# felixchenfy/Monocular-Visual-Odometry

Measured on AMD Instinct MI355X. Metric: frames/sec (extract+match+5-kf BA), 640x480 / 2000 kp, 1->8 MI355X, higher is better.
Workload: dtype u8 (extract/match) + f64 (BA); 1 GPU

## Files before the change

### include/mvo_hip.h

```cpp
#ifndef MVO_HIP_H
#define MVO_HIP_H
#include <stdint.h>

#ifdef __cplusplus
extern "C" {
#endif

#define MVO_OK 0
#define MVO_ERR_INVALID (-1)
#define MVO_ERR_NO_DEVICE (-2)
#define MVO_ERR_CAPACITY (-3)
#define MVO_ERR_HIP (-4)
#define MVO_ERR_STATE (-5)

typedef struct mvo_ctx mvo_ctx;

typedef struct {
    float x, y, size, angle, response;
    int32_t octave, class_id;
} mvo_keypoint;

typedef struct {
    int32_t queryIdx, trainIdx, imgIdx;
    float distance;
// ... 206 lines not shown
    double R[9], t[3], T_w_c[16], mean_depth, scale;
    double mean_pixel_dist, mean_angle, median_angle, min_angle, max_angle;
    int criteria[3], good;
} mvo_init_result;
int mvo_init_two_view(mvo_ctx* ctx, const float* pts1, const float* pts2, int n, double fx, double fy, double cx,
                      double cy, double prob, double threshold, double h_threshold, double h_confidence, double sigma,
                      const double* T_w_c_ref, const mvo_init_params* params, mvo_init_poses* poses,
                      mvo_init_result* out);
int mvo_retain_good_triangulation(const float* pts3d_in_curr, int n, const double* T_w_c_curr, const double* T_w_c_ref,
                                  double min_triang_angle, double max_ratio_to_median, int32_t* keep, int* n_keep,
                                  double* angles);
int mvo_rodrigues(const double* rvec, double* R);
int mvo_invert_pose(const double* T, double* T_inv);

int mvo_ba_launch_stats(int device, long long* launches, long long* windows, double* ms, int reset);
int mvo_debug_ba_service_times(int device, double* out5);
int mvo_debug_ba_resident_stats(int device, long long* windows, long long* grid_starts);
int mvo_debug_ba_resident_cycles(int device, double* shader_cycles);
int mvo_debug_ba_path_switches(int device, long long* n);
int mvo_debug_ba_demand_replay(const double* times, int n, uint8_t* decisions);
int mvo_profile_enable(mvo_ctx* ctx, int on);
int mvo_profile_reset(mvo_ctx* ctx);
typedef struct {
    char name[48];
    int64_t launches;
    double total_ms;
} mvo_kernel_time;
int mvo_profile_get(mvo_ctx* ctx, mvo_kernel_time* out, int cap);

int mvo_debug_set(const char* key, int value);
int mvo_debug_ba_trace_enable(mvo_ctx* ctx, int on);
int mvo_debug_get_ba_trace(mvo_ctx* ctx, mvo_ba_handle* handle, double* rows, int cap, int* n);
int mvo_debug_get_ba_plan(mvo_ctx* ctx, mvo_ba_handle* handle, int* wgs, int* nsplit, int32_t* wg_pt_start, int cap);
int mvo_debug_get_ba_phases(mvo_ctx* ctx, long long* cycles, int n, int* wgs);
int mvo_debug_get_level(mvo_ctx* ctx, int level, int blurred, uint8_t* out, int cap, int* w, int* h, int* stride);
int mvo_debug_get_candidates(mvo_ctx* ctx, void* out, int cap, int* n);
int mvo_debug_get_undistort_map(mvo_ctx* ctx, int32_t* ix, int32_t* iy, uint8_t* ax, uint8_t* ay, int cap);

int mvo_debug_get_pnp(mvo_ctx* ctx, double* models, int32_t* counts, int cap, int32_t* info);

int mvo_debug_get_essential(mvo_ctx* ctx, int32_t* counts, int cap_iters, int32_t* info);

int mvo_debug_get_homography(mvo_ctx* ctx, int32_t* counts, int cap_iters, int32_t* info);

int mvo_debug_get_recover_pose(mvo_ctx* ctx, int32_t* good, int32_t* chosen, double* R1R2t, uint8_t* masks, int cap);
int mvo_debug_get_homography_decomposition(mvo_ctx* ctx, double* Hn, double* w, int32_t* branch, double* Rs,
                                           double* ts, double* normals, int32_t* rejected);
int mvo_debug_get_init_finish(mvo_ctx* ctx, float* p_curr, double* cosang, double* pixdist, int cap, int* n);

#ifdef __cplusplus
}
#endif
#endif
```

### monocular-visual-odometry_amd/__init__.py

```python
import ctypes as C
import os

import numpy as np

from . import synth

_HERE = os.path.dirname(os.path.abspath(__file__))
LIB_PATH = os.path.join(_HERE, "csrc", "libmvo_hip.so")
HEADER_PATH = os.path.join(os.path.dirname(_HERE), "include", "mvo_hip.h")

MVO_OK, MVO_ERR_INVALID, MVO_ERR_NO_DEVICE, MVO_ERR_CAPACITY, MVO_ERR_HIP, MVO_ERR_STATE = 0, -1, -2, -3, -4, -5

KEYPOINT_DTYPE = np.dtype([("x", "<f4"), ("y", "<f4"), ("size", "<f4"), ("angle", "<f4"),
                           ("response", "<f4"), ("octave", "<i4"), ("class_id", "<i4")])
DMATCH_DTYPE = np.dtype([("queryIdx", "<i4"), ("trainIdx", "<i4"), ("imgIdx", "<i4"), ("distance", "<f4")])
CANDIDATE_DTYPE = np.dtype([("x", "<i2"), ("y", "<i2"), ("level_score", "<i4"), ("harris", "<f4"), ("angle", "<f4")])
DISTRIBUTE_CANDIDATE_DTYPE = np.dtype([("x", "<i4"), ("y", "<i4"), ("level", "<i4"), ("score", "<i4")])


class OrbParams(C.Structure):
    _fields_ = [("nfeatures", C.c_int32), ("scale_factor", C.c_float), ("nlevels", C.c_int32),
                ("fast_threshold", C.c_int32), ("max_keypoints", C.c_int32), ("grid_size", C.c_int32),
                ("grid_max_per_cell", C.c_int32), ("pyramid_interpolation", C.c_int32)]

# ... 456 lines not shown

    def ba_solve_batch(self, problems, **kw):
        prs = (BaProblem * len(problems))()
        keeps = []
        for i, a in enumerate(problems):
            d = dict(info=(1, 0, 0, 1), huber_delta=1.0, fix_points=False, pose_fixed=None, max_iterations=50)
            d.update(kw)
            pr, keep = self._ba_problem(*a, d["info"], d["huber_delta"], d["fix_points"], d["pose_fixed"], d["max_iterations"])
            prs[i] = pr
            keeps.append(keep)
        sts = (BaStats * len(problems))()
        self._chk(self.lib.mvo_ba_solve_batch(self.h, prs, len(problems), sts))
        return [(k["poses"].reshape(-1, 4, 4), k["points"], {f: getattr(sts[i], f) for f, _ in BaStats._fields_})
                for i, k in enumerate(keeps)]

    def ba_set_mode(self, mode):
        self._chk(self.lib.mvo_ba_set_mode(self.h, {"latency": 0, "throughput": 1, "shared": 2}[mode]))

    def ba_trace_enable(self, on=True):
        self._chk(self.lib.mvo_debug_ba_trace_enable(self.h, int(on)))

    def ba_trace(self, handle=None, raw_rows=0):
        out = np.zeros((512, 4))
        n = C.c_int()
        self._chk(self.lib.mvo_debug_get_ba_trace(self.h, handle[0] if handle else None, _p(out),
                                                  -int(raw_rows) if raw_rows else 512, C.byref(n)))
        return out[:n.value].copy()

    def ba_plan(self, handle=None):
        g, ns = C.c_int(), C.c_int()
        pt = np.zeros(257, np.int32)
        self._chk(self.lib.mvo_debug_get_ba_plan(self.h, handle[0] if handle else None, C.byref(g), C.byref(ns), _p(pt), 257))
        return dict(wgs=g.value, nsplit=ns.value & 0xffff, groups=max(1, ns.value >> 16), wg_pt_start=pt[:g.value + 1].copy())

    def map_create(self):
        m = C.c_void_p()
        self._chk(self.lib.mvo_map_create(self.h, C.byref(m)))
        return m

    def map_release(self, m):
        self.lib.mvo_map_release.restype = None
        self.lib.mvo_map_release(self.h, m)

    def map_upload(self, m, pos, desc):
        pos = np.ascontiguousarray(pos, np.float32).reshape(-1, 3)
        desc = np.ascontiguousarray(desc, np.uint8).reshape(-1, 32)
        assert len(pos) == len(desc)
        self._chk(self.lib.mvo_map_upload(self.h, m, _p(pos), _p(desc), len(pos)))

    def map_update_positions(self, m, pos, first=0):
        pos = np.ascontiguousarray(pos, np.float32).reshape(-1, 3)
        self._chk(self.lib.mvo_map_update_positions(self.h, m, _p(pos), int(first), len(pos)))

    def map_points_in_view(self, m, T_w_c, K, cols, rows, cap):
        T = np.ascontiguousarray(T_w_c, np.float64).reshape(4, 4)
        idx = np.zeros(max(cap, 1), np.int32)
        px = np.zeros((max(cap, 1), 2), np.float32)
        n = C.c_int()
        d = C.c_void_p()
        self._chk(self.lib.mvo_map_points_in_view(self.h, m, _p(T), C.c_double(K["fx"]), C.c_double(K["fy"]),
                                                  C.c_double(K["cx"]), C.c_double(K["cy"]), int(cols), int(rows),
                                                  _p(idx), _p(px), int(cap), C.byref(n), C.byref(d)))
        return idx[:n.value].copy(), px[:n.value].copy(), d.value

    def solve_pnp_ransac(self, pts3d, pts2d, K, iterations=100, reprojection_error=2.0, confidence=0.999):
        p3 = np.ascontiguousarray(pts3d, np.float32).reshape(-1, 3)
# ... 435 lines not shown
```

### monocular-visual-odometry_amd/csrc/ba_host.cpp

```cpp
#include <algorithm>
#include <atomic>
#include <cmath>
#include <cstdio>
#include <condition_variable>
#include <cstdlib>
#include <cstring>
#include <chrono>
#include <deque>
#include <map>
#include <mutex>
#include <thread>
#include <vector>

#include "ba_types.h"
#include "mvo_internal.h"

int ba_kernel_set_lds_limit();
hipError_t ba_kernel_launch(const BaBatch& batch, int max_wgs, size_t lds_bytes, hipStream_t stream, int profile, int nr, int slots);
int ba_solver_class(int n);
hipError_t ba_service_launch(const BaServiceArgs& a, hipStream_t stream);

void ba_service_free(int device, void* p, bool host);

int g_ba_use_mfma = 1;
// ... 5 lines not shown
int g_ba_service = 1;
int g_ba_edge_rows = -1;
int g_ba_uv_global = std::getenv("MVO_BA_UV_GLOBAL") ? std::atoi(std::getenv("MVO_BA_UV_GLOBAL")) : 1;
int g_ba_chunk_pieces = 0;
int g_ba_block_solver = 0;
int g_ba_groups = std::getenv("MVO_BA_GROUPS") ? std::atoi(std::getenv("MVO_BA_GROUPS")) : 1;
int g_ba_alias_sl = std::getenv("MVO_BA_ALIAS_SL") ? std::atoi(std::getenv("MVO_BA_ALIAS_SL")) : 1;

struct BaDemand {
    double t[128] = {0}, flip = -1e9, low_since = -1, last = 0, rate_avg = 0;
    long long n = 0, total = 0, flips = 0;
    bool on = false;
    bool submit(double now);
};

namespace {

struct Carver {
    size_t off = 0;
    size_t take(size_t bytes) {
        size_t o = off;
        off = (off + bytes + 255) / 256 * 256;
        return o;
    }
};

struct BaPlan {
    int F = 0, L = 0, E = 0, G = 1, nfree = 0, n = 0, NT = 1, npair = 1, nlow = 0, npk = 16, slice = 0, nsplit = 1, npar = 1, nseq = 1,
        ldu = 16, nhp = 1, maxEg = 0, maxLg = 0, max_dup = 0, fix_points = 0, e2_edges = 0, slots = 1, npt = 1, panel = 0, uv_global = 0,
        alias_sl = 0, groups = 1;
    bool service = false;
    size_t uarea = 0;
    size_t lds = 0;
    std::vector<int> wg_pt;
    size_t o_desc = 0, o_pin = 0, o_ptsin = 0, o_wpt = 0, o_wed = 0, o_wps = 0, o_ep = 0, o_el = 0, o_uv = 0, o_ptstart = 0,
           o_ptl = 0, o_eof = 0, o_dup = 0, o_slot = 0, o_sp = 0, o_pkt = 0, upload_end = 0, x_end = 0;
    size_t o_uvd = 0, o_dxl = 0, o_stats = 0, o_pout = 0, o_pts = 0, o_xp = 0, o_xr = 0, o_xh = 0, o_xc = 0, total = 0;
    size_t m_stats = 0, m_poses = 0, m_pts = 0, m_trace = 0, pin_total = 0;
    bool runnable = true;
};

struct BaWorkspace {
    int device = 0;
    char* dev = nullptr;
    size_t dev_cap = 0;
    char* pin = nullptr;
    size_t pin_cap = 0;
    unsigned seq = 0;
    size_t x_sig[5] = {0, 0, 0, 0, 0};
    hipEvent_t ready = nullptr;
    BaPlan plan;
    bool in_flight = false;
    bool poisoned = false;
};

int ws_reserve(mvo_ctx* ctx, BaWorkspace& ws, size_t dev_bytes, size_t pin_bytes) {
    ws.device = ctx->device;
    if (ws.poisoned) {
        ws.dev = ws.pin = nullptr;
        ws.dev_cap = ws.pin_cap = 0;
        ws.seq = 0;
        std::memset(ws.x_sig, 0, sizeof ws.x_sig);
        ws.poisoned = false;
    }
    if (!ws.ready) MVO_HIP(hipEventCreateWithFlags(&ws.ready, hipEventDisableTiming));
    if (dev_bytes > ws.dev_cap) {
// ... 703 lines not shown
                P.panel = (n + 1 > 32 || g_ba_block_solver) ? 1 : 0;
                uarea = ba_uarea_doubles(do_schur ? 4 * npar * msplit : 0, ldu, pt_edges, maxEpose, nhp, G, p->fix_points);
                const bool uv_may_be_global = !all_lds && maxEg > BA_THREADS && g_ba_uv_global;
                for (int uvg = 0; uvg <= (uv_may_be_global ? 1 : 0) && !fits; ++uvg) {
                    P.uv_global = uvg;
                    P.alias_sl = (do_schur && npar == 1 && g_ba_alias_sl && uarea >= ba_solver_matrix_doubles(n, nlow + nhp, G, npair, npar)) ? 1 : 0;
                    P.lds = ba_lds_bytes(F, n, nlow, nhp, G, npair, npar, nfree, maxEg, maxLg, p->fix_points, uarea, P.e2_edges, P.panel, P.uv_global,
                                         P.alias_sl);
                    fits = P.lds <= BA_LDS_BUDGET;
                }
                if (plan_trace)
                    std::fprintf(stderr, "[mvo plan] G %d rows_in_lds %d chunks %d pieces %d pt_passes %d maxEg %d maxLg %d uarea %zu B lds %zu B (budget %d) %s\n",
                                 G, all_lds, nseq, npar, P.npt, maxEg, maxLg, uarea * 8, P.lds, BA_LDS_BUDGET, fits ? "fits" : "-");
                if (all_lds && g_ba_edge_rows != 0) {
                    if (uarea < (size_t)BA_MSTRIDE * (maxEg + 2 * F)) fits = false;
                    break;
                }
            }
        }
        if (fits && maxEg <= BA_EDGE_SLOTS * BA_THREADS && maxLg < 32000) break;
        if (G >= BA_MAX_WGS)
            return mvo_set_err(ctx, MVO_ERR_CAPACITY, "BA window too large for the LDS-resident solver", hipSuccess);
        {
            int next = BA_MAX_WGS;
            for (int c : {2, 4, 8, 16, 32, 64, 128, 256, per_xcd / 2, per_xcd, 2 * per_xcd, 4 * per_xcd, 8 * per_xcd})
                if (c > G && c < next) next = c;
            G = next;
        }
    }
    g_stage_times.lap(0);
    P.nsplit = nsplit;
    P.npar = npar;
    P.nseq = nseq;
    P.uarea = uarea;
    P.G = G;
    P.maxEg = maxEg;
    P.maxLg = maxLg;
    P.groups = 1;
    if (G > 32 && g_ba_groups) {
        int K = 2;
        while (G / K > 32 && K < 8) K *= 2;
        if (G % K == 0 && G / K <= 32 && uarea >= (size_t)K * (size_t)(nlow + nhp)) P.groups = K;
    }
    P.slice = (nlow + G / P.groups - 1) / (G / P.groups);
    std::vector<int>&e_pose = SC.e_pose, &e_point = SC.e_point, &ptstart = SC.ptstart, &ptlist = SC.ptlist;
    std::vector<double>& e_uv = SC.e_uv;
    e_pose.resize(E);
    e_point.resize(E);
    ptstart.assign(L + 1, 0);
    ptlist.resize(E);
    e_uv.resize(2 * (size_t)E);
    {
        std::vector<int>& cur = SC.cur;
        cur.resize((size_t)G * std::max(F, 1));
        for (int g = 0; g < G; ++g)
            for (int q = 0; q < F; ++q) cur[(size_t)g * F + q] = wg_pose[(size_t)g * (F + 1) + q];
        for (int e : act) {
            const int k = cur[(size_t)owner[p->edge_point[e]] * F + p->edge_pose[e]]++;
            e_pose[k] = p->edge_pose[e];
            e_point[k] = p->edge_point[e];
            e_uv[2 * (size_t)k] = p->edge_uv[2 * (size_t)e];
            e_uv[2 * (size_t)k + 1] = p->edge_uv[2 * (size_t)e + 1];
        }
    }
    for (int k = 0; k < E; ++k) ptstart[e_point[k] + 1]++;
    for (int i = 0; i < L; ++i) ptstart[i + 1] += ptstart[i];
    {
        std::vector<int>& cur = SC.cur2;
        cur.assign(ptstart.begin(), ptstart.end() - 1);
        for (int k = 0; k < E; ++k) ptlist[cur[e_point[k]]++] = k;
    }
    std::vector<short>&eof = SC.eof, &dup = SC.dup;
    eof.assign((size_t)std::max(L, 1) * std::max(nfree, 1), -1);
    dup.assign(std::max(E, 1), 0);
    int max_dup = 0;
// ... 346 lines not shown
int ba_fetch_device(mvo_ctx* ctx, mvo_ba_handle* H, double* poses, double* points, mvo_ba_stats* st) {
    if (H->ws.plan.runnable) {
        if (!H->launched) return mvo_set_err(ctx, MVO_ERR_STATE, "mvo_ba_fetch without mvo_ba_solve_resident", hipSuccess);
        service_wait(service_for(ctx->device), &H->job, 1);
        H->launched = false;
    }
    return ba_collect(ctx, H->ws, H->job, poses, points, st);
}
void ba_release_device(mvo_ctx* ctx, mvo_ba_handle* H) {
    if (!H) return;
    if (H->launched) service_wait(service_for(ctx ? ctx->device : H->ws.device), &H->job, 1);
    ws_free(H->ws);
    delete H;
}

int ba_get_trace(mvo_ctx* ctx, mvo_ba_handle* H, double* rows, int cap, int* n) {
    BaWorkspace* ws = H ? &H->ws : (ctx->ba_pool && !ctx->ba_pool->ws.empty() ? ctx->ba_pool->ws[0] : nullptr);
    if (!ws || !ws->pin) return mvo_set_err(ctx, MVO_ERR_STATE, "no bundle adjustment has run", hipSuccess);
    const BaStatsDev* s = (const BaStatsDev*)(ws->pin + ws->plan.m_stats);
    const int m = cap < 0 ? std::min(-cap, BA_TRACE_MAX) : std::min(std::min(s->trials, BA_TRACE_MAX), cap);
    if (rows) std::memcpy(rows, ws->pin + ws->plan.m_trace, (size_t)m * sizeof(BaTraceRow));
    if (n) *n = m;
    return MVO_OK;
}
int ba_get_plan(mvo_ctx* ctx, mvo_ba_handle* H, int* G, int* nsplit, int32_t* wg_pt, int cap) {
    BaWorkspace* ws = H ? &H->ws : (ctx->ba_pool && !ctx->ba_pool->ws.empty() ? ctx->ba_pool->ws[0] : nullptr);
    if (!ws) return mvo_set_err(ctx, MVO_ERR_STATE, "no bundle adjustment has been planned", hipSuccess);
    if (G) *G = ws->plan.G;
    if (nsplit) *nsplit = ws->plan.nsplit | (ws->plan.groups > 1 ? ws->plan.groups << 16 : 0);
    if (wg_pt)
        for (int i = 0; i <= ws->plan.G && i < cap; ++i) wg_pt[i] = ws->plan.wg_pt[i];
    return MVO_OK;
}
void ba_service_times(int device, double* out5) {
    for (int i = 0; i < 5; ++i) out5[i] = 0;
    if (device < 0 || device >= 16) return;
    BaService* sp;
    {
        std::lock_guard<std::mutex> lk(*g_service_start);
        sp = g_service[device & 15];
    }
    if (!sp) return;
    std::lock_guard<std::mutex> lk(sp->m);
    out5[0] = sp->t_idle, out5[1] = sp->t_batch, out5[2] = sp->t_launch, out5[3] = sp->t_sync, out5[4] = sp->t_post;
}
void ba_service_park(int device) {
    if (device < 0 || device >= 16) return;
    BaService* sp;
    {
        std::lock_guard<std::mutex> lk(*g_service_start);
        sp = g_service[device & 15];
    }
    if (!sp) return;
    std::unique_lock<std::mutex> lk(sp->m);
    if (!sp->resident) return;
    sp->park_requested = true;
    sp->cv_work.notify_all();
    sp->cv_done.wait_for(lk, std::chrono::milliseconds(50), [&] { return !sp->resident || sp->slots_busy > 0 || !sp->q.empty(); });
}
void ba_resident_stats(int device, long long* windows, long long* grid_starts, double* cycles, long long* path_switches) {
    if (windows) *windows = 0;
    if (grid_starts) *grid_starts = 0;
    if (cycles) *cycles = 0;
    if (path_switches) *path_switches = 0;
    if (device < 0 || device >= 16) return;
    BaService* sp;
// ... 43 lines not shown
```

### monocular-visual-odometry_amd/csrc/ba_kernels.hip

```cpp
#include "ba_types.h"
#include "mvo_internal.h"

typedef ba_u64 u64;
#ifndef MVO_KERNEL_SIM
typedef __attribute__((address_space(1))) double gdouble;
typedef __attribute__((address_space(1))) const u64 gcu64;
typedef __attribute__((address_space(1))) u64 gu64;
#define BA_AS_GLOBAL_D(p) ((gdouble*)(p))
#define BA_AS_GLOBAL_CU64(p) ((gcu64*)(p))
#define BA_AS_GLOBAL_U64(p) ((gu64*)(p))
#else
typedef double gdouble;
typedef const u64 gcu64;
typedef u64 gu64;
#define BA_AS_GLOBAL_D(p) (p)
#define BA_AS_GLOBAL_CU64(p) (p)
#define BA_AS_GLOBAL_U64(p) (p)
#endif

#define PH_BEGIN() long long ph_t = PROF ? (long long)__builtin_amdgcn_s_memtime() : 0
#define PH_END(id)                                                       \
    do {                                                                 \
        if (PROF) {                                                      \
            long long ph_n = (long long)__builtin_amdgcn_s_memtime();    \
// ... 794 lines not shown
    if (do_schur && wave < B.npair * npar) {
#pragma unroll
        for (int j = 0; j < 4; ++j) pk4[j] = pkt_g[(wave % B.npair) * 256 + ((lane >> 4) + 4 * j) * 16 + (lane & 15)];
    }
    EdgeRegs er;
#pragma unroll
    for (int c = 0; c < 6; ++c) er.a0[c] = er.a1[c] = er.x[c] = 0;
    const bool have0 = SLOTS > 0 && tid < Eg, have1 = SLOTS > 1 && tid + BA_THREADS < Eg;
    const int e0_p = have0 ? W.epose[tid] : 0, e0_l = have0 ? W.ept[tid] : 0, e0_sl = have0 ? sSlot[e0_p] : -1;
    constexpr int nslot = SLOTS;
    constexpr int e2_first = SLOTS == 0 ? 0 : BA_THREADS;
#define BA_EDGE_FROM_LDS(BODY, el_)                                          \
    do {                                                                     \
        EdgeRegs r1_;                                                        \
        double ee_[2];                                                       \
        const double* q_ = W.E2 + BA_E2S * ((el_)-e2_first);                 \
        _Pragma("unroll") for (int c_ = 0; c_ < 6; ++c_) {                   \
            r1_.a0[c_] = q_[c_];                                             \
            r1_.a1[c_] = q_[6 + c_];                                         \
            r1_.x[c_] = q_[12 + c_];                                         \
        }                                                                    \
        ee_[0] = q_[18];                                                     \
        ee_[1] = q_[19];                                                     \
        const int p1_ = W.epose[el_];                                        \
        (void)p1_;                                                           \
        BODY(el_, r1_, W.ept[el_], sSlot[p1_], ee_)                          \
    } while (0);
#define BA_EDGES(BODY)                                                       \
    if (nslot > 0 && have0) do { BODY(tid, er, e0_l, e0_sl, ee0) } while (0); \
    if (nslot > 1 && have1) BA_EDGE_FROM_LDS(BODY, tid + BA_THREADS)         \
    if (nslot == 0)                                                          \
        for (int el0_ = tid; el0_ < Eg; el0_ += BA_THREADS) BA_EDGE_FROM_LDS(BODY, el0_)

    int hp_npass = 1;
    {
        const int mcap = (int)(B.uarea / BA_MSTRIDE);
        for (;; ++hp_npass) {
            int tot = 0;
            for (int p = 0; p < B.F; ++p) {
                const int n_p = sPoseStart[p + 1] - sPoseStart[p];
                tot += min(n_p, ((n_p + hp_npass - 1) / hp_npass + 1) & ~1);
            }
            if (tot <= mcap) break;
            if (hp_npass > Eg) {
                error = 1;
                break;
            }
        }
    }
    const bool hp_tables = hp_npass <= BA_HP_PASSES;
    auto hp_slice_row = [&](int q, int row) {
        if (tid < B.F) {
            int off = 0, lo = 0, hi = 0;
            for (int pp = 0; pp <= tid; ++pp) {
                const int s0 = sPoseStart[pp], n_p = sPoseStart[pp + 1] - s0;
                const int h = ((n_p + hp_npass - 1) / hp_npass + 1) & ~1;
                off += hi - lo;
                lo = min(s0 + q * h, s0 + n_p);
                hi = min(s0 + (q + 1) * h, s0 + n_p);
            }
            sSlc[0][row][tid] = (short)lo;
            sSlc[1][row][tid] = (short)hi;
            sSlc[2][row][tid] = (short)off;
        }
    };
    if (hp_tables && !error)
        for (int q = 0; q < hp_npass; ++q) hp_slice_row(q, q);
    int nfp = 0, hp_pa0 = -1, hp_pb0 = -1, hp_pa1 = -1, hp_pb1 = -1;
    for (int p = 0; p < B.F; ++p) {
        if (sSlot[p] < 0) continue;
        if (nfp == 2 * wave) hp_pa0 = p;
        if (nfp == 2 * wave + 1) hp_pb0 = p;
        if (nfp == 2 * (wave + BA_WAVES)) hp_pa1 = p;
        if (nfp == 2 * (wave + BA_WAVES) + 1) hp_pb1 = p;
        ++nfp;
    }
    __syncthreads();

    int piv_hoff = 0;
    if (NR == 32 && n > 0) {
        const int lsh = NR == 32 ? 4 : (n <= 32 ? 4 : (n <= 64 ? 3 : 2)), LPR = 1 << lsh, jj = tid & (LPR - 1);
        const int qi = min(tid >> lsh, n - 1), q0 = min(jj, n - 1), q1 = min(jj + LPR, n - 1);
        piv_hoff = (36 * sSlotPose[qi / 6] + 7 * (qi % 6)) | (36 * sSlotPose[q0 / 6] + 7 * (q0 % 6)) << 10 | (36 * sSlotPose[q1 / 6] + 7 * (q1 % 6)) << 20;
    }
    for (it = 0; any_free && !error && it < B.max_it; ++it) {
        PH_BEGIN();
        BA_PHASE_HEAD();
        double ee0[2] = {0, 0};
// ... 80 lines not shown
                    for (int i = 0; i < 6; ++i) W.Hll[BA_XS * l + i] = h6[i];
#pragma unroll
                    for (int i = 0; i < 3; ++i) W.bl[3 * l + i] = b[i];
                    maxdiag = fmax(maxdiag, fmax(fabs(h6[0]), fmax(fabs(h6[3]), fabs(h6[5]))));
                }
                __syncthreads();
            }
        }
        PH_END(2);
        const bool hp_deferred = do_schur && G > 1 && it > 0;
        const bool hp_local = hp_deferred || G == 1;
        if (!hp_deferred) ++tagH;
        BA_PHASE_HEAD();
        {
            const int col = lane & 15;
            v4d accp0 = {0, 0, 0, 0}, accp1 = {0, 0, 0, 0};
            for (int q = 0; q < hp_npass && !error; ++q) {
                const int tq = hp_tables ? q : 0;
                if (!hp_tables) {
                    hp_slice_row(q, 0);
                    __syncthreads();
                }
#define BA_BODY_STAGE_M(el, r, l_, sl_, ee)                                   \
    const int p_ = W.epose[el];                                              \
    const int lo_ = sSlc[0][tq][p_], hi_ = sSlc[1][tq][p_];                  \
    if ((el) < lo_ || (el) >= hi_) break;                                    \
    double* Mr = stage + BA_MSTRIDE * (sSlc[2][tq][p_] + (el)-lo_);          \
    _Pragma("unroll") for (int c = 0; c < 6; ++c) {                          \
        Mr[c] = r.a0[c];                                                     \
        Mr[7 + c] = r.a1[c];                                                 \
    }                                                                        \
    Mr[6] = ee[0];                                                           \
    Mr[13] = ee[1];
                BA_EDGES(BA_BODY_STAGE_M)
                __syncthreads();
                const bool lastq = q == hp_npass - 1;
                if (batch.use_mfma) {
                    int ai = 0;
                    for (int pair = wave; 2 * pair < nfp; pair += BA_WAVES, ++ai) {
                        const int pa = ai == 0 ? hp_pa0 : hp_pa1, pb = ai == 0 ? hp_pb0 : hp_pb1;
                        const bool second = col >= 8;
                        const int pp = second ? pb : pa;
                        const int cc7 = col & 7;
                        const bool cv = cc7 < 7 && pp >= 0;
                        const int rowsA = 2 * (sSlc[1][tq][pa] - sSlc[0][tq][pa]);
                        const int rowsB = pb >= 0 ? 2 * (sSlc[1][tq][pb] - sSlc[0][tq][pb]) : 0;
                        const int s = pp >= 0 ? sSlc[2][tq][pp] : 0, rows = second ? rowsB : rowsA;
                        const int rmax = max(rowsA, rowsB);
                        const double* pm = stage + BA_MSTRIDE * (s + (lane >> 5)) + 7 * ((lane >> 4) & 1) + (cv ? cc7 : 0);
                        const int kq = lane >> 4;
                        const int myrows = cv ? rows - kq : 0;
                        v4d acc = ai == 0 ? accp0 : accp1;
                        int st = 0;
#define BA_HP_LOAD4(V)                                                                   \
    V##0 = 4 * st < myrows ? pm[0] : 0.0, V##1 = 4 * st + 4 < myrows ? pm[2 * BA_MSTRIDE] : 0.0, \
    V##2 = 4 * st + 8 < myrows ? pm[4 * BA_MSTRIDE] : 0.0, V##3 = 4 * st + 12 < myrows ? pm[6 * BA_MSTRIDE] : 0.0; \
    pm += 8 * BA_MSTRIDE;                                                                \
    st += 4
#define BA_HP_MFMA4_LOADNEXT(V, Wn, more)                                      \
    acc = __builtin_amdgcn_mfma_f64_16x16x4f64(V##0, V##0, acc, 0, 0, 0);       \
    __builtin_amdgcn_sched_barrier(0);                                          \
    if (more) { BA_HP_LOAD4(Wn); }                                              \
    __builtin_amdgcn_sched_barrier(0);                                          \
    acc = __builtin_amdgcn_mfma_f64_16x16x4f64(V##1, V##1, acc, 0, 0, 0);       \
    acc = __builtin_amdgcn_mfma_f64_16x16x4f64(V##2, V##2, acc, 0, 0, 0);       \
    acc = __builtin_amdgcn_mfma_f64_16x16x4f64(V##3, V##3, acc, 0, 0, 0)
                        if (4 * (st + 4) <= rmax) {
                            double a0, a1, a2, a3, c0 = 0, c1 = 0, c2 = 0, c3 = 0;
                            BA_HP_LOAD4(a);
                            for (;;) {
                                const bool more1 = 4 * (st + 4) <= rmax;
                                BA_HP_MFMA4_LOADNEXT(a, c, more1);
                                if (!more1) break;
                                const bool more2 = 4 * (st + 4) <= rmax;
                                BA_HP_MFMA4_LOADNEXT(c, a, more2);
                                if (!more2) break;
                            }
                        }
#undef BA_HP_LOAD4
#undef BA_HP_MFMA4_LOADNEXT
                        for (; 4 * st < rmax; ++st) {
                            const double v = 4 * st < myrows ? pm[0] : 0.0;
                            acc = __builtin_amdgcn_mfma_f64_16x16x4f64(v, v, acc, 0, 0, 0);
                            pm += 2 * BA_MSTRIDE;
                        }
                        if (ai == 0) accp0 = acc;
                        else accp1 = acc;
                        if (lastq) {
#pragma unroll
                            for (int j = 0; j < 4; ++j) {
                                const int rg = (lane >> 4) + 4 * j;
                                const bool mine = second ? (rg >= 8 && rg < 15 && pb >= 0) : rg < 7;
                                const int r7 = rg & 7;
                                if (mine && cc7 <= r7 && cc7 < 7) {
                                    const int sl = sSlot[pp], pk = r7 * (r7 + 1) / 2 + cc7;
                                    if (hp_local) W.hpl[BA_HP * sl + pk] = acc[j];
                                    else gstore_d(B.xH + 2 * ((size_t)g * B.nhp + BA_HP * sl + pk), tag0 + tagH, acc[j], same_l2);
                                }
                            }
                        }
                    }
                } else {
                    for (int p = wave; p < B.F; p += BA_WAVES) {
                        const int sl = sSlot[p];
                        if (sl < 0 || lane >= BA_HP) continue;
                        const int lo = sSlc[0][tq][p], hi = sSlc[1][tq][p];
                        const int s = sSlc[2][tq][p], e = s + hi - lo;
                        int i = 0;
                        while ((i + 1) * (i + 2) / 2 <= lane) ++i;
                        const int j = lane - i * (i + 1) / 2;
                        double acc = q == 0 ? 0.0 : W.hpl[BA_HP * sl + lane];
                        for (int r = 2 * s; r < 2 * e; ++r)
                            acc = __builtin_fma(stage[BA_MSTRIDE * (r >> 1) + 7 * (r & 1) + i], stage[BA_MSTRIDE * (r >> 1) + 7 * (r & 1) + j], acc);
                        if (hp_local || !lastq) W.hpl[BA_HP * sl + lane] = acc;
                        else gstore_d(B.xH + 2 * ((size_t)g * B.nhp + BA_HP * sl + lane), tag0 + tagH, acc, same_l2);
                    }
                }
                __syncthreads();
            }
        }
        PH_END(1);
        BA_PHASE_HEAD();
        if (!hp_deferred) {
            const double m = block_max(maxdiag, sScr);
            const int nhp = B.nhp, hrows = min(G, max(1, (int)(B.uarea / nhp)));
            double hsum = 0, mm = 0;
            if (G > 1) {
                if (tid == 0) gstore_d(B.xH + 2 * ((size_t)g * nhp + nhp - 1), tag0 + tagH, m, same_l2);
                for (int w0 = 0; w0 < G; w0 += hrows) {
                    const int nr = min(hrows, G - w0);
                    if (!gather_tagged(B.xH + 2 * (size_t)w0 * nhp, nr * nhp, nhp, nhp, tag0 + tagH, stage)) sFlag[2] = 1;
                    __syncthreads();
                    if (tid < nhp - 1) {
#pragma unroll 8
                        for (int w = 0; w < nr; ++w) hsum += stage[w * nhp + tid];
                    }
                    if (tid < nr) mm = fmax(mm, stage[tid * nhp + nhp - 1]);
                    __syncthreads();
                }
                if (sFlag[2]) error = 1;
            } else {
                if (tid < nhp - 1) hsum = W.hpl[tid];
                if (tid == 0) mm = m;
            }
            if (tid < BA_HP * nfree) {
                const int sl = tid / BA_HP, pk = tid - BA_HP * sl, p = sSlotPose[sl];
// ... 734 lines not shown
```

### monocular-visual-odometry_amd/csrc/ba_types.h

```cpp
#ifndef MVO_BA_TYPES_H
#define MVO_BA_TYPES_H
#include <stddef.h>
#include <stdint.h>

typedef unsigned long long ba_u64;

#define BA_THREADS 512
#define BA_WAVES 8
#define BA_MAX_POSES 20
#define BA_MSTRIDE 15
#define BA_XS 7
#define BA_SXS 9
#define BA_EDGE_SLOTS 2
#define BA_PANEL_DOUBLES 1040
#define BA_E2S 21
#define BA_LDS_BUDGET (157 * 1024)
#define BA_MAX_WGS 256
#define BA_MAX_BATCH 16
#define BA_NPHASE 16
#define BA_TRACE_MAX 512
#define BA_HP_PASSES 6
#define BA_HP 28

struct BaStatsDev {
// ... 85 lines not shown
    ba_u64* cmd;
    ba_u64* arrived;
    ba_u64 first_seq[BA_SERVICE_SLOTS];
    int nslots, wgs_per_slot;
};

__host__ __device__ inline size_t ba_solver_matrix_doubles(int n, int nlow, int G, int npair, int npar) {
    size_t a = n + 1 <= 32 ? 32 * 33 : (n + 1 <= 64 ? 64 * 65 : (size_t)(n + 1) * (size_t)(n + 2));
    const size_t sp = (size_t)npair * (size_t)(npar > 1 ? npar - 1 : 0) * 256;
    const size_t sl = (size_t)((nlow + G - 1) / (G > 0 ? G : 1)) * (size_t)G;
    if (sp > a) a = sp;
    if (sl > a) a = sl;
    return a;
}
__host__ __device__ inline size_t ba_solver_doubles(int n, int nlow, int G, int npair, int npar, int panel, int alias = 0) {
    return (alias ? 0 : ba_solver_matrix_doubles(n, nlow, G, npair, npar)) + 3 * 64 +
           (panel ? BA_PANEL_DOUBLES : 0);
}
__host__ __device__ inline size_t ba_pose_doubles(int F) { return (size_t)(F > 0 ? F : 1) * 82; }
__host__ __device__ inline size_t ba_uarea_doubles(int ucols, int ldu, int max_pt_edges, int maxEpose, int nhp, int G, int fix_points) {
    size_t hrows = 4096 / (size_t)(nhp > 0 ? nhp : 1);
    if (hrows < 1) hrows = 1;
    if (hrows > (size_t)G) hrows = (size_t)G;
    size_t a = (size_t)nhp * hrows;
    const size_t m = (size_t)BA_MSTRIDE * (size_t)(maxEpose > 0 ? maxEpose : 1);
    if (m > a) a = m;
    if (!fix_points) {
        const size_t u = (size_t)ucols * (size_t)(ldu + 1), sx = (size_t)BA_SXS * max_pt_edges;
        if (u > a) a = u;
        if (sx > a) a = sx;
    }
    return a;
}
__host__ __device__ inline size_t ba_lds_bytes(int F, int n, int nlow, int nhp, int G, int npair, int npar, int nfree, int maxEg,
                                               int maxLg, int fix_points, size_t uarea, int e2_edges, int panel, int uv_global = 0,
                                               int alias_sl = 0) {
    size_t d = ba_solver_doubles(n, nlow + nhp, G, npair, npar, panel, alias_sl) + (size_t)nlow + 2 * (size_t)nhp + 17 +
               (uv_global ? 0 : (size_t)maxEg * 2) + (size_t)maxLg * 3;
    d += ba_pose_doubles(F) + 2 * (size_t)G + 8;
    if (!fix_points) d += (size_t)maxLg * (3 + BA_XS + 3 + BA_XS + 3);
    d += uarea + (size_t)e2_edges * BA_E2S;
    size_t shorts = (size_t)maxEg * 5 + (size_t)maxLg + 1 + (size_t)maxLg * (nfree > 0 ? nfree : 1);
    return d * 8 + ((shorts * 2 + 15) & ~(size_t)15) + 64;
}

#endif
```

### monocular-visual-odometry_amd/csrc/mvo_api_ba.cpp

```cpp
#include <cstring>

#include "mvo_internal.h"

int ba_demand_replay(const double* times, int n, unsigned char* decisions);
extern int g_ba_use_mfma, g_ba_wgs, g_ba_same_l2, g_ba_profile, g_ba_block_solver, g_ba_cu_share, g_ba_xcd_reserve, g_ba_edge_rows, g_ba_service, g_ba_chunk_pieces, g_ba_uv_global, g_ba_alias_sl;
int ba_debug_set(const char* key, int value) {
    if (!std::strcmp(key, "ba_mfma")) g_ba_use_mfma = value;
    else if (!std::strcmp(key, "ba_profile")) g_ba_profile = value;
    else if (!std::strcmp(key, "ba_same_l2")) g_ba_same_l2 = value;
    else if (!std::strcmp(key, "ba_wgs")) g_ba_wgs = value;
    else if (!std::strcmp(key, "ba_block_solver")) g_ba_block_solver = value;
    else if (!std::strcmp(key, "ba_cu_share")) g_ba_cu_share = value;
    else if (!std::strcmp(key, "ba_xcd_reserve")) g_ba_xcd_reserve = value;
    else if (!std::strcmp(key, "ba_edge_rows")) g_ba_edge_rows = value;
    else if (!std::strcmp(key, "ba_service")) g_ba_service = value;
    else if (!std::strcmp(key, "ba_chunk_pieces")) g_ba_chunk_pieces = value;
    else if (!std::strcmp(key, "ba_uv_global")) g_ba_uv_global = value;
    else if (!std::strcmp(key, "ba_alias_sl")) g_ba_alias_sl = value;
    else return MVO_ERR_INVALID;
    return MVO_OK;
}

extern "C" {

// ... 79 lines not shown
}

int mvo_debug_ba_path_switches(int device, long long* n) {
    if (!n) return MVO_ERR_INVALID;
    ba_resident_stats(device, nullptr, nullptr, nullptr, n);
    return MVO_OK;
}

int mvo_debug_ba_resident_cycles(int device, double* shader_cycles) {
    if (!shader_cycles) return MVO_ERR_INVALID;
    ba_resident_stats(device, nullptr, nullptr, shader_cycles);
    return MVO_OK;
}

int mvo_ba_launch_stats(int device, long long* launches, long long* windows, double* ms, int reset) {
    if (device < 0 || device > 15) return MVO_ERR_INVALID;
    ba_launch_stats(device, launches, windows, ms, reset);
    return MVO_OK;
}
int mvo_debug_ba_trace_enable(mvo_ctx* ctx, int on) {
    if (!ctx) return MVO_ERR_INVALID;
    ba_set_trace(ctx, on);
    return MVO_OK;
}
int mvo_debug_get_ba_trace(mvo_ctx* ctx, mvo_ba_handle* handle, double* rows, int cap, int* n) {
    if (!ctx) return MVO_ERR_INVALID;
    return ba_get_trace(ctx, handle, rows, cap, n);
}
int mvo_debug_get_ba_plan(mvo_ctx* ctx, mvo_ba_handle* handle, int* wgs, int* nsplit, int32_t* wg_pt_start, int cap) {
    if (!ctx) return MVO_ERR_INVALID;
    return ba_get_plan(ctx, handle, wgs, nsplit, wg_pt_start, cap);
}

int mvo_debug_ba_demand_replay(const double* times, int n, uint8_t* decisions) {
    if (!times || !decisions || n < 0) return MVO_ERR_INVALID;
    return ba_demand_replay(times, n, decisions);
}

int mvo_debug_get_ba_phases(mvo_ctx* ctx, long long* cycles, int n, int* wgs) {
    if (!ctx || !cycles) return MVO_ERR_INVALID;
    for (int i = 0; i < n && i < 16; ++i) cycles[i] = ctx->ba_phase[i];
    if (wgs) *wgs = ctx->ba_wgs;
    return MVO_OK;
}

}
```

### monocular-visual-odometry_amd/csrc/mvo_internal.h

```cpp
#ifndef MVO_INTERNAL_H
#define MVO_INTERNAL_H
#include <hip/hip_runtime.h>
#include <stdint.h>

#ifndef MVO_KERNEL_SIM
#define MVO_DYN_LDS(T, name) extern __shared__ T name[]
#define MVO_DYN_LDS_ALIGNED16(T, name) extern __shared__ __attribute__((aligned(16))) T name[]
#define MVO_WAVES_PER_EU(lo, hi) __attribute__((amdgpu_waves_per_eu(lo, hi)))
#define MVO_WAIT_VM0() asm volatile("s_waitcnt vmcnt(0)" ::: "memory")
#define MVO_OPAQUE(x) asm volatile("" : "+v"(x))
#else
#define MVO_DYN_LDS(T, name) T* name = static_cast<T*>(emu_dyn_lds())
#define MVO_DYN_LDS_ALIGNED16(T, name) T* name = static_cast<T*>(emu_dyn_lds())
#define MVO_WAVES_PER_EU(lo, hi)
#define MVO_WAIT_VM0() __atomic_thread_fence(__ATOMIC_SEQ_CST)
#define MVO_OPAQUE(x) (void)(x)
#endif

#include <chrono>
#include <cstdio>
#include <cstdlib>
#include <map>
#include <atomic>
#include <string>
// ... 369 lines not shown
int epipolar_launch_knn2(mvo_ctx* ctx, const uint8_t* d_q, const float* d_qxy, int nq, const uint8_t* d_t, const float* d_txy,
                         const double* d_tol2, int nt, const EpipolarArgs& a, unsigned long long* d_part, int32_t* d_part_cnt,
                         int32_t* d_arrive, int32_t* out);
int projection_groups(int nt);
int projection_launch(mvo_ctx* ctx, const float* d_pos, const uint8_t* d_desc, int n_map, const TrackViewArgs& a, const uint8_t* d_t,
                      const double* d_tg, int nt, unsigned long long* d_part, int32_t* d_part_cnt, int32_t* d_arrive, int32_t* out);
int dist_launch_cells(mvo_ctx* ctx, const DistCell* d_cells, int n_cells, int thr_min, int thr_ini, int32_t* counts,
                      DistRecord* records);
int dist_launch_ic_angle(mvo_ctx* ctx, const signed char* d_disc, int disc_n, const DistRecord* kps, int n, float* angles);
extern int g_pyr_force_chain;
extern int g_match_mfma;
extern int g_pnp_replay_skew;
void track_release(mvo_ctx* ctx);
struct TrackInitView {
    const float *kp1, *kp2, *pts;
    const int32_t* lists;
    const double *e_out, *h_out;
    uint8_t* out;
};
int track_init_view(mvo_ctx* ctx, int n, int m, TrackInitView* v);
struct mvo_ba_handle;
int ba_solve_device(mvo_ctx* ctx, mvo_ba_problem* p, mvo_ba_stats* st);
int ba_begin_device(mvo_ctx* ctx, const mvo_ba_problem* p);
int ba_end_device(mvo_ctx* ctx, mvo_ba_problem* p, mvo_ba_stats* st);
int ba_solve_batch_device(mvo_ctx* ctx, mvo_ba_problem* ps, int n, mvo_ba_stats* sts);
int ba_prepare_device(mvo_ctx* ctx, const mvo_ba_problem* p, mvo_ba_handle** out);
int ba_run_device(mvo_ctx* ctx, mvo_ba_handle* H);
int ba_fetch_device(mvo_ctx* ctx, mvo_ba_handle* H, double* poses, double* points, mvo_ba_stats* st);
void ba_release_device(mvo_ctx* ctx, mvo_ba_handle* H);
void ba_pool_release(mvo_ctx* ctx);
void ba_set_trace(mvo_ctx* ctx, int on);
int ba_get_trace(mvo_ctx* ctx, mvo_ba_handle* H, double* rows, int cap, int* n);
int ba_get_plan(mvo_ctx* ctx, mvo_ba_handle* H, int* G, int* nsplit, int32_t* wg_pt, int cap);
void ba_launch_stats(int device, long long* launches, long long* windows, double* ms, int reset);
void ba_service_times(int device, double* out5);
void ba_service_park(int device);
void ba_resident_stats(int device, long long* windows, long long* grid_starts, double* cycles = nullptr, long long* path_switches = nullptr);
void ba_service_free(int device, void* p, bool host);
inline void mvo_free_on_current_device(void* p) {
    int d = 0;
    (void)hipGetDevice(&d);
    ba_service_free(d, p, false);
}

#endif
```

Measured before the change: 5628 frames/s.

## Stage only first-slot edges for pose Hessian blocks, read second slot from E2

When the BA kernel runs with two edge slots, it now stages only the first-slot edges (up to BA_THREADS) into the LDS staging area for pose-block Hessian accumulation. Second-slot edges are read directly from the per-edge E2 buffer on the last pass, in both the MFMA and scalar paths. The host planner enlarges the staging area to hold one slot's worth of rows when LDS fits, and computes the pass count with a shared host/device helper. The goal is fewer staging passes and fewer redundant staging writes, at the cost of extra branching in the MFMA row loads and scattered global/E2 reads.

```diff
diff --git a/include/mvo_hip.h b/include/mvo_hip.h
--- a/include/mvo_hip.h
+++ b/include/mvo_hip.h
@@ -262,6 +262,7 @@
 int mvo_debug_ba_trace_enable(mvo_ctx* ctx, int on);
 int mvo_debug_get_ba_trace(mvo_ctx* ctx, mvo_ba_handle* handle, double* rows, int cap, int* n);
 int mvo_debug_get_ba_plan(mvo_ctx* ctx, mvo_ba_handle* handle, int* wgs, int* nsplit, int32_t* wg_pt_start, int cap);
+int mvo_debug_get_ba_hp_passes(mvo_ctx* ctx, mvo_ba_handle* handle, int* passes, int* staged_edges);
 int mvo_debug_get_ba_phases(mvo_ctx* ctx, long long* cycles, int n, int* wgs);
 int mvo_debug_get_level(mvo_ctx* ctx, int level, int blurred, uint8_t* out, int cap, int* w, int* h, int* stride);
 int mvo_debug_get_candidates(mvo_ctx* ctx, void* out, int cap, int* n);
diff --git a/monocular-visual-odometry_amd/__init__.py b/monocular-visual-odometry_amd/__init__.py
--- a/monocular-visual-odometry_amd/__init__.py
+++ b/monocular-visual-odometry_amd/__init__.py
@@ -512,6 +512,11 @@
         pt = np.zeros(257, np.int32)
         self._chk(self.lib.mvo_debug_get_ba_plan(self.h, handle[0] if handle else None, C.byref(g), C.byref(ns), _p(pt), 257))
         return dict(wgs=g.value, nsplit=ns.value & 0xffff, groups=max(1, ns.value >> 16), wg_pt_start=pt[:g.value + 1].copy())
+
+    def ba_hp_passes(self, handle=None):
+        n, e = C.c_int(), C.c_int()
+        self._chk(self.lib.mvo_debug_get_ba_hp_passes(self.h, handle[0] if handle else None, C.byref(n), C.byref(e)))
+        return n.value, e.value
 
     def map_create(self):
         m = C.c_void_p()
diff --git a/monocular-visual-odometry_amd/csrc/ba_host.cpp b/monocular-visual-odometry_amd/csrc/ba_host.cpp
--- a/monocular-visual-odometry_amd/csrc/ba_host.cpp
+++ b/monocular-visual-odometry_amd/csrc/ba_host.cpp
@@ -61,6 +61,7 @@
     bool service = false;
     size_t uarea = 0;
     size_t lds = 0;
+    int hp_passes = 1, hp_staged = 0;
     std::vector<int> wg_pt;
     size_t o_desc = 0, o_pin = 0, o_ptsin = 0, o_wpt = 0, o_wed = 0, o_wps = 0, o_ep = 0, o_el = 0, o_uv = 0, o_ptstart = 0,
            o_ptl = 0, o_eof = 0, o_dup = 0, o_slot = 0, o_sp = 0, o_pkt = 0, upload_end = 0, x_end = 0;
@@ -830,7 +831,23 @@
     P.nsplit = nsplit;
     P.npar = npar;
     P.nseq = nseq;
+    const size_t plan_area = uarea;
+    if (P.slots == 2 && ba_uarea_hp_doubles(uarea) > uarea) {
+        const size_t lds = ba_lds_bytes(F, n, nlow, nhp, G, npair, npar, nfree, maxEg, maxLg, p->fix_points, ba_uarea_hp_doubles(uarea), P.e2_edges, P.panel,
+                                        P.uv_global, P.alias_sl);
+        if (lds <= BA_LDS_BUDGET) {
+            uarea = ba_uarea_hp_doubles(uarea);
+            P.lds = lds;
+        }
+        if (plan_trace) std::fprintf(stderr, "[mvo plan] pose-block staging: uarea %zu B lds %zu B %s\n", ba_uarea_hp_doubles(plan_area) * 8, lds, lds <= BA_LDS_BUDGET ? "fits" : "-");
+    }
     P.uarea = uarea;
+    P.hp_passes = 1, P.hp_staged = 0;
+    for (int g = 0; g < G; ++g) {
+        int staged = 0;
+        P.hp_passes = std::max(P.hp_passes, ba_hp_passes(&wg_pose[(size_t)g * (F + 1)], F, wg_edge[g], P.slots, uarea, &staged));
+        P.hp_staged = std::max(P.hp_staged, staged);
+    }
     P.G = G;
     P.maxEg = maxEg;
     P.maxLg = maxLg;
@@ -838,7 +855,7 @@
     if (G > 32 && g_ba_groups) {
         int K = 2;
         while (G / K > 32 && K < 8) K *= 2;
-        if (G % K == 0 && G / K <= 32 && uarea >= (size_t)K * (size_t)(nlow + nhp)) P.groups = K;
+        if (G % K == 0 && G / K <= 32 && plan_area >= (size_t)K * (size_t)(nlow + nhp)) P.groups = K;
     }
     P.slice = (nlow + G / P.groups - 1) / (G / P.groups);
     std::vector<int>&e_pose = SC.e_pose, &e_point = SC.e_point, &ptstart = SC.ptstart, &ptlist = SC.ptlist;
@@ -1251,6 +1268,13 @@
         for (int i = 0; i <= ws->plan.G && i < cap; ++i) wg_pt[i] = ws->plan.wg_pt[i];
     return MVO_OK;
 }
+int ba_get_hp_passes(mvo_ctx* ctx, mvo_ba_handle* H, int* passes, int* staged_edges) {
+    BaWorkspace* ws = H ? &H->ws : (ctx->ba_pool && !ctx->ba_pool->ws.empty() ? ctx->ba_pool->ws[0] : nullptr);
+    if (!ws) return mvo_set_err(ctx, MVO_ERR_STATE, "no bundle adjustment has been planned", hipSuccess);
+    if (passes) *passes = ws->plan.hp_passes;
+    if (staged_edges) *staged_edges = ws->plan.hp_staged;
+    return MVO_OK;
+}
 void ba_service_times(int device, double* out5) {
     for (int i = 0; i < 5; ++i) out5[i] = 0;
     if (device < 0 || device >= 16) return;
diff --git a/monocular-visual-odometry_amd/csrc/ba_kernels.hip b/monocular-visual-odometry_amd/csrc/ba_kernels.hip
--- a/monocular-visual-odometry_amd/csrc/ba_kernels.hip
+++ b/monocular-visual-odometry_amd/csrc/ba_kernels.hip
@@ -850,28 +850,19 @@
     if (nslot == 0)                                                          \
         for (int el0_ = tid; el0_ < Eg; el0_ += BA_THREADS) BA_EDGE_FROM_LDS(BODY, el0_)
 
-    int hp_npass = 1;
-    {
-        const int mcap = (int)(B.uarea / BA_MSTRIDE);
-        for (;; ++hp_npass) {
-            int tot = 0;
-            for (int p = 0; p < B.F; ++p) {
-                const int n_p = sPoseStart[p + 1] - sPoseStart[p];
-                tot += min(n_p, ((n_p + hp_npass - 1) / hp_npass + 1) & ~1);
-            }
-            if (tot <= mcap) break;
-            if (hp_npass > Eg) {
-                error = 1;
-                break;
-            }
-        }
+    constexpr int hp_slots = SLOTS;
+    int hp_npass = ba_hp_passes(sPoseStart, B.F, 0, hp_slots, (size_t)B.uarea, nullptr);
+    if (hp_npass == 0) {
+        hp_npass = 1;
+        error = 1;
     }
     const bool hp_tables = hp_npass <= BA_HP_PASSES;
     auto hp_slice_row = [&](int q, int row) {
         if (tid < B.F) {
             int off = 0, lo = 0, hi = 0;
             for (int pp = 0; pp <= tid; ++pp) {
-                const int s0 = sPoseStart[pp], n_p = sPoseStart[pp + 1] - s0;
+                const int s0 = hp_slots == 2 ? min(sPoseStart[pp], BA_THREADS) : sPoseStart[pp];
+                const int n_p = ba_hp_staged(sPoseStart[pp], sPoseStart[pp + 1], hp_slots);
                 const int h = ((n_p + hp_npass - 1) / hp_npass + 1) & ~1;
                 off += hi - lo;
                 lo = min(s0 + q * h, s0 + n_p);
@@ -1018,9 +1009,14 @@
     }                                                                        \
     Mr[6] = ee[0];                                                           \
     Mr[13] = ee[1];
-                BA_EDGES(BA_BODY_STAGE_M)
+                if (hp_slots == 2) {
+                    if (have0) do { BA_BODY_STAGE_M(tid, er, e0_l, e0_sl, ee0) } while (0);
+                } else {
+                    BA_EDGES(BA_BODY_STAGE_M)
+                }
                 __syncthreads();
                 const bool lastq = q == hp_npass - 1;
+                const bool hp_e2 = hp_slots == 2 && lastq;
                 if (batch.use_mfma) {
                     int ai = 0;
                     for (int pair = wave; 2 * pair < nfp; pair += BA_WAVES, ++ai) {
@@ -1029,19 +1025,26 @@
                         const int pp = second ? pb : pa;
                         const int cc7 = col & 7;
                         const bool cv = cc7 < 7 && pp >= 0;
-                        const int rowsA = 2 * (sSlc[1][tq][pa] - sSlc[0][tq][pa]);
-                        const int rowsB = pb >= 0 ? 2 * (sSlc[1][tq][pb] - sSlc[0][tq][pb]) : 0;
+                        const int stgA = sSlc[1][tq][pa] - sSlc[0][tq][pa];
+                        const int stgB = pb >= 0 ? sSlc[1][tq][pb] - sSlc[0][tq][pb] : 0;
+                        const int e2A = hp_e2 ? max(sPoseStart[pa], e2_first) : 0;
+                        const int e2B = hp_e2 && pb >= 0 ? max(sPoseStart[pb], e2_first) : 0;
+                        const int rowsA = 2 * (stgA + (hp_e2 ? max(sPoseStart[pa + 1] - e2A, 0) : 0));
+                        const int rowsB = 2 * (stgB + (hp_e2 && pb >= 0 ? max(sPoseStart[pb + 1] - e2B, 0) : 0));
                         const int s = pp >= 0 ? sSlc[2][tq][pp] : 0, rows = second ? rowsB : rowsA;
                         const int rmax = max(rowsA, rowsB);
                         const double* pm = stage + BA_MSTRIDE * (s + (lane >> 5)) + 7 * ((lane >> 4) & 1) + (cv ? cc7 : 0);
                         const int kq = lane >> 4;
                         const int myrows = cv ? rows - kq : 0;
+                        const int mystg = (second ? stgB : stgA) - (lane >> 5);
+                        int pe = BA_E2S * ((second ? e2B : e2A) - e2_first - mystg) + (cc7 == 6 ? 18 + ((lane >> 4) & 1) : 6 * ((lane >> 4) & 1) + (cv ? cc7 : 0));
                         v4d acc = ai == 0 ? accp0 : accp1;
                         int st = 0;
+#define BA_HP_ROW(k) (4 * st + 4 * (k) < myrows ? *(hp_slots == 2 && 2 * st + 2 * (k) >= mystg ? W.E2 + (pe + 2 * (k) * BA_E2S) : pm + 2 * (k) * BA_MSTRIDE) : 0.0)
 #define BA_HP_LOAD4(V)                                                                   \
-    V##0 = 4 * st < myrows ? pm[0] : 0.0, V##1 = 4 * st + 4 < myrows ? pm[2 * BA_MSTRIDE] : 0.0, \
-    V##2 = 4 * st + 8 < myrows ? pm[4 * BA_MSTRIDE] : 0.0, V##3 = 4 * st + 12 < myrows ? pm[6 * BA_MSTRIDE] : 0.0; \
+    V##0 = BA_HP_ROW(0), V##1 = BA_HP_ROW(1), V##2 = BA_HP_ROW(2), V##3 = BA_HP_ROW(3);   \
     pm += 8 * BA_MSTRIDE;                                                                \
+    pe += 8 * BA_E2S;                                                                    \
     st += 4
 #define BA_HP_MFMA4_LOADNEXT(V, Wn, more)                                      \
     acc = __builtin_amdgcn_mfma_f64_16x16x4f64(V##0, V##0, acc, 0, 0, 0);       \
@@ -1066,10 +1069,12 @@
 #undef BA_HP_LOAD4
 #undef BA_HP_MFMA4_LOADNEXT
                         for (; 4 * st < rmax; ++st) {
-                            const double v = 4 * st < myrows ? pm[0] : 0.0;
+                            const double v = BA_HP_ROW(0);
                             acc = __builtin_amdgcn_mfma_f64_16x16x4f64(v, v, acc, 0, 0, 0);
                             pm += 2 * BA_MSTRIDE;
+                            pe += 2 * BA_E2S;
                         }
+#undef BA_HP_ROW
                         if (ai == 0) accp0 = acc;
                         else accp1 = acc;
                         if (lastq) {
@@ -1098,6 +1103,13 @@
                         double acc = q == 0 ? 0.0 : W.hpl[BA_HP * sl + lane];
                         for (int r = 2 * s; r < 2 * e; ++r)
                             acc = __builtin_fma(stage[BA_MSTRIDE * (r >> 1) + 7 * (r & 1) + i], stage[BA_MSTRIDE * (r >> 1) + 7 * (r & 1) + j], acc);
+                        if (hp_e2) {
+                            const int x0 = max(sPoseStart[p], e2_first) - e2_first, x1 = sPoseStart[p + 1] - e2_first;
+                            for (int r = 2 * x0; r < 2 * x1; ++r) {
+                                const double* er2 = W.E2 + BA_E2S * (r >> 1);
+                                acc = __builtin_fma(i < 6 ? er2[6 * (r & 1) + i] : er2[18 + (r & 1)], j < 6 ? er2[6 * (r & 1) + j] : er2[18 + (r & 1)], acc);
+                            }
+                        }
                         if (hp_local || !lastq) W.hpl[BA_HP * sl + lane] = acc;
                         else gstore_d(B.xH + 2 * ((size_t)g * B.nhp + BA_HP * sl + lane), tag0 + tagH, acc, same_l2);
                     }
diff --git a/monocular-visual-odometry_amd/csrc/ba_types.h b/monocular-visual-odometry_amd/csrc/ba_types.h
--- a/monocular-visual-odometry_amd/csrc/ba_types.h
+++ b/monocular-visual-odometry_amd/csrc/ba_types.h
@@ -141,6 +141,31 @@
     }
     return a;
 }
+#define BA_HP_STAGE_EDGES BA_THREADS
+__host__ __device__ inline int ba_hp_staged(int s0, int e0, int slots) {
+    if (slots != 2) return e0 - s0;
+    return (e0 < BA_THREADS ? e0 : BA_THREADS) - (s0 < BA_THREADS ? s0 : BA_THREADS);
+}
+__host__ __device__ inline int ba_hp_passes(const int* pose_start, int F, int base, int slots, size_t uarea, int* staged_out) {
+    const int mcap = (int)(uarea / BA_MSTRIDE), Eg = pose_start[F] - pose_start[0];
+    int staged = 0;
+    for (int p = 0; p < F; ++p) staged += ba_hp_staged(pose_start[p] - base, pose_start[p + 1] - base, slots);
+    if (staged_out) *staged_out = staged;
+    for (int npass = 1;; ++npass) {
+        int tot = 0;
+        for (int p = 0; p < F; ++p) {
+            const int n_p = ba_hp_staged(pose_start[p] - base, pose_start[p + 1] - base, slots);
+            const int h = ((n_p + npass - 1) / npass + 1) & ~1;
+            tot += n_p < h ? n_p : h;
+        }
+        if (tot <= mcap) return npass;
+        if (npass > Eg) return 0;
+    }
+}
+__host__ __device__ inline size_t ba_uarea_hp_doubles(size_t uarea) {
+    const size_t m = (size_t)BA_MSTRIDE * BA_HP_STAGE_EDGES;
+    return uarea > m ? uarea : m;
+}
 __host__ __device__ inline size_t ba_lds_bytes(int F, int n, int nlow, int nhp, int G, int npair, int npar, int nfree, int maxEg,
                                                int maxLg, int fix_points, size_t uarea, int e2_edges, int panel, int uv_global = 0,
                                                int alias_sl = 0) {
diff --git a/monocular-visual-odometry_amd/csrc/mvo_api_ba.cpp b/monocular-visual-odometry_amd/csrc/mvo_api_ba.cpp
--- a/monocular-visual-odometry_amd/csrc/mvo_api_ba.cpp
+++ b/monocular-visual-odometry_amd/csrc/mvo_api_ba.cpp
@@ -135,6 +135,11 @@
     return ba_get_plan(ctx, handle, wgs, nsplit, wg_pt_start, cap);
 }
 
+int mvo_debug_get_ba_hp_passes(mvo_ctx* ctx, mvo_ba_handle* handle, int* passes, int* staged_edges) {
+    if (!ctx) return MVO_ERR_INVALID;
+    return ba_get_hp_passes(ctx, handle, passes, staged_edges);
+}
+
 int mvo_debug_ba_demand_replay(const double* times, int n, uint8_t* decisions) {
     if (!times || !decisions || n < 0) return MVO_ERR_INVALID;
     return ba_demand_replay(times, n, decisions);
diff --git a/monocular-visual-odometry_amd/csrc/mvo_internal.h b/monocular-visual-odometry_amd/csrc/mvo_internal.h
--- a/monocular-visual-odometry_amd/csrc/mvo_internal.h
+++ b/monocular-visual-odometry_amd/csrc/mvo_internal.h
@@ -425,6 +425,7 @@
 void ba_set_trace(mvo_ctx* ctx, int on);
 int ba_get_trace(mvo_ctx* ctx, mvo_ba_handle* H, double* rows, int cap, int* n);
 int ba_get_plan(mvo_ctx* ctx, mvo_ba_handle* H, int* G, int* nsplit, int32_t* wg_pt, int cap);
+int ba_get_hp_passes(mvo_ctx* ctx, mvo_ba_handle* H, int* passes, int* staged_edges);
 void ba_launch_stats(int device, long long* launches, long long* windows, double* ms, int reset);
 void ba_service_times(int device, double* out5);
 void ba_service_park(int device);
```

Result: faster. 5695 frames/s, median of 6 (+1.2%).
